# Kronuz/Xapiand

Hardware: AMD Instinct MI355X
Metric: queries/sec + p50 latency, 10M-doc synthetic index, 3-term AND, top-10 (higher is better)
Workload: dtype u32 postings + f64 BM25

## Files before the change

### include/xgm.h

```cpp
#ifndef XGM_H
#define XGM_H

#include <stddef.h>
#include <stdint.h>

#ifdef __cplusplus
extern "C" {
#endif
#if defined(__GNUC__)
#pragma GCC visibility push(default)
#endif

#define XGM_MAX_TERMS 16
#define XGM_MAX_K 1024

#define XGM_OK 0
#define XGM_UNSUPPORTED 1
#define XGM_E_INVALID (-1)
#define XGM_E_IO (-2)
#define XGM_E_NO_DEVICE (-3)
#define XGM_E_DEVICE (-4)
#define XGM_E_REVISION (-5)
#define XGM_E_NOMEM (-6)

// ... 326 lines not shown
void xgm_batch_release(xgm_inflight*);

int xgm_merge_shards_device(xgm_index*, const void* d_all_hits, const void* d_all_hdrs,
                            uint32_t n_shards, uint32_t nq, uint32_t k_stride, const uint32_t* k,
                            void* d_out_hits, void* d_out_hdrs);

size_t xgm_shard_record_bytes(uint32_t nq, uint32_t k_stride);
int xgm_merge_shards_packed_device(xgm_index*, const void* d_all_records, uint32_t n_shards, uint32_t nq, uint32_t k_stride,
                                   const uint32_t* k, void* d_out_hits, void* d_out_hdrs);

int xgm_search_sharded(xgm_index* const* shards, uint32_t n_shards, const xgm_query_desc* descs,
                       uint32_t nq, uint32_t k_stride, xgm_hit* hits, xgm_result_hdr* hdrs);

int xgm_debug_sharded_info(const xgm_index* shards0, uint64_t* out4);

int xgm_index_set_near_colocated(xgm_index*, int may_exist);

int xgm_index_set_profiling(xgm_index*, int on);
double xgm_last_kernel_ms(const xgm_index*);
const char* xgm_last_kernel_name(const xgm_index*);

#define XGM_TRAFFIC_FIELDS 10
int xgm_last_batch_traffic(xgm_index*, uint64_t* out, uint32_t n);

uint64_t xgm_query_postings_bytes(const xgm_index*, const xgm_query*);

int64_t xgm_debug_decode_term_device(xgm_index*, uint32_t term_id, uint32_t* did, uint32_t* wdf, uint64_t cap);

int64_t xgm_debug_read_doclen(xgm_index*, uint32_t* out, uint64_t cap);

int64_t xgm_debug_read_positions(xgm_index*, uint32_t term_id, uint32_t* out, uint64_t cap);

int64_t xgm_debug_read_container(xgm_index*, uint32_t term_id, uint32_t stripe, unsigned char* out, uint64_t cap, uint32_t* layout);

int xgm_debug_read_wdf_summary(xgm_index*, uint32_t term_id, uint32_t stripe, uint64_t* out);

int xgm_debug_read_term_wdf0(xgm_index*, uint32_t term_id, uint32_t* out);

int64_t xgm_debug_read_flat(xgm_index*, uint32_t term_id, uint32_t* did, unsigned char* wdf, uint32_t* pos, uint64_t cap, uint32_t* has_pos);

double xgm_debug_plan_us(const xgm_index*, const xgm_query_desc* descs, const xgm_global_stats* gs, uint32_t nq, uint32_t reps);

int xgm_debug_batch_launches(const xgm_index*, const xgm_query* qs, uint32_t nq, char* out, uint32_t cap);

int xgm_debug_host_ns(uint64_t* out8);

// ... 32 lines not shown
```

### xapiand_amd/_lib.py

```python
import ctypes as C
import os

XGM_MAX_TERMS = 16
XGM_MAX_TREE = 40
XGM_OP_TREE = 8
XGM_MAX_K = 1024
XGM_OK, XGM_UNSUPPORTED = 0, 1
XGM_E_INVALID, XGM_E_IO, XGM_E_NO_DEVICE, XGM_E_DEVICE, XGM_E_REVISION, XGM_E_NOMEM = -1, -2, -3, -4, -5, -6
XGM_OP_AND, XGM_OP_OR, XGM_OP_PHRASE = 1, 2, 3
XGM_OP_AND_NOT, XGM_OP_AND_MAYBE, XGM_OP_FILTER, XGM_OP_NEAR = 4, 5, 6, 7
XGM_REPLAY_BATCH_COUNT = 2
XGM_REPLAY_BATCH_FROZEN = 1
XGM_KNOWN_LOWER_BOUND = 1 << 63
XGM_ALL_NOT_A_MATCH = 0x80000000
XGM_MATCHES_LOWER_BOUND = 1 << 63
XGM_DEVICE_NONE = -1
UINT64_MAX = (1 << 64) - 1

_HERE = os.path.dirname(os.path.abspath(__file__))
LIB_PATH = os.environ.get("XGM_LIB_PATH") or os.path.join(_HERE, "csrc", "libxgm.so")


class RawPostings(C.Structure):
    _fields_ = [("n_terms", C.c_uint32), ("lastdocid", C.c_uint32), ("doccount", C.c_uint32),
# ... 156 lines not shown
    ("xgm_debug_replay_list", C.c_int, [C.c_int, _P(Hit), C.c_uint64, C.c_uint32, C.c_uint64, C.c_uint32, C.c_uint64, _P(Hit), _P(ReplayFigures)]),
    ("xgm_debug_batch_replay_info", C.c_int, [_P(C.c_uint64)]),
    ("xgm_search_batch", C.c_int, [C.c_void_p, _P(Query), C.c_uint32, C.c_uint32, _P(Hit), _P(ResultHdr)]),
    ("xgm_search_batch_known", C.c_int, [C.c_void_p, _P(Query), C.c_uint32, C.c_uint32, _P(Hit), _P(ResultHdr), _P(C.c_uint64)]),
    ("xgm_search_batch_begin", C.c_int, [C.c_void_p, _P(Query), C.c_uint32, C.c_uint32, _P(C.c_void_p)]),
    ("xgm_get_mset_batch_begin", C.c_int, [C.c_void_p, _P(QueryDesc), _P(GlobalStats), C.c_uint32, C.c_uint32, _P(C.c_void_p)]),
    ("xgm_batch_end", C.c_int, [C.c_void_p, _P(_P(Hit)), _P(_P(ResultHdr))]),
    ("xgm_batch_known", C.c_int, [C.c_void_p, _P(_P(C.c_uint64))]),
    ("xgm_batch_poll", C.c_int, [C.c_void_p]),
    ("xgm_batch_release", None, [C.c_void_p]),
    ("xgm_search_batch_device", C.c_int, [C.c_void_p, _P(Query), C.c_uint32, C.c_uint32, C.c_void_p, C.c_void_p]),
    ("xgm_get_mset_batch", C.c_int, [C.c_void_p, _P(QueryDesc), _P(GlobalStats), C.c_uint32, C.c_uint32, _P(Hit), _P(ResultHdr)]),
    ("xgm_get_mset_batch_device", C.c_int, [C.c_void_p, _P(QueryDesc), _P(GlobalStats), C.c_uint32, C.c_uint32, C.c_void_p, C.c_void_p]),
    ("xgm_search_sharded", C.c_int, [_P(C.c_void_p), C.c_uint32, _P(QueryDesc), C.c_uint32, C.c_uint32, _P(Hit), _P(ResultHdr)]),
    ("xgm_debug_sharded_info", C.c_int, [C.c_void_p, _P(C.c_uint64)]),
    ("xgm_merge_shards_device", C.c_int, [C.c_void_p, C.c_void_p, C.c_void_p, C.c_uint32, C.c_uint32, C.c_uint32, _P(C.c_uint32), C.c_void_p, C.c_void_p]),
    ("xgm_merge_shards_packed_device", C.c_int, [C.c_void_p, C.c_void_p, C.c_uint32, C.c_uint32, C.c_uint32, _P(C.c_uint32), C.c_void_p, C.c_void_p]),
    ("xgm_shard_record_bytes", C.c_size_t, [C.c_uint32, C.c_uint32]),
    ("xgm_index_set_profiling", C.c_int, [C.c_void_p, C.c_int]),
    ("xgm_index_set_near_colocated", C.c_int, [C.c_void_p, C.c_int]),
    ("xgm_last_kernel_ms", C.c_double, [C.c_void_p]),
    ("xgm_last_kernel_name", C.c_char_p, [C.c_void_p]),
    ("xgm_last_batch_traffic", C.c_int, [C.c_void_p, _P(C.c_uint64), C.c_uint32]),
    ("xgm_query_postings_bytes", C.c_uint64, [C.c_void_p, _P(Query)]),
    ("xgm_debug_decode_term_device", C.c_int64, [C.c_void_p, C.c_uint32, _P(C.c_uint32), _P(C.c_uint32), C.c_uint64]),
    ("xgm_debug_read_doclen", C.c_int64, [C.c_void_p, _P(C.c_uint32), C.c_uint64]),
    ("xgm_debug_read_positions", C.c_int64, [C.c_void_p, C.c_uint32, _P(C.c_uint32), C.c_uint64]),
    ("xgm_debug_read_container", C.c_int64, [C.c_void_p, C.c_uint32, C.c_uint32, _P(C.c_ubyte), C.c_uint64, _P(C.c_uint32)]),
    ("xgm_debug_read_wdf_summary", C.c_int, [C.c_void_p, C.c_uint32, C.c_uint32, _P(C.c_uint64)]),
    ("xgm_debug_read_term_wdf0", C.c_int, [C.c_void_p, C.c_uint32, _P(C.c_uint32)]),
    ("xgm_debug_read_flat", C.c_int64, [C.c_void_p, C.c_uint32, _P(C.c_uint32), _P(C.c_ubyte), _P(C.c_uint32), C.c_uint64, _P(C.c_uint32)]),
    ("xgm_debug_plan_us", C.c_double, [C.c_void_p, _P(QueryDesc), _P(GlobalStats), C.c_uint32, C.c_uint32]),
    ("xgm_debug_batch_launches", C.c_int, [C.c_void_p, _P(Query), C.c_uint32, C.c_char_p, C.c_uint32]),
    ("xgm_index_set_batching", C.c_int, [C.c_void_p, C.c_uint32]),
    ("xgm_debug_batching_info", C.c_int, [C.c_void_p, _P(C.c_uint64)]),
    ("xgm_debug_host_ns", C.c_int, [_P(C.c_uint64)]),
    ("xgm_debug_concurrent_searches", C.c_double, [C.c_void_p, _P(QueryDesc), _P(GlobalStats), C.c_uint32, C.c_uint32, C.c_uint32, C.c_uint32, _P(C.c_double)]),
    ("xgm_debug_phase_cycles", C.c_int, [_P(C.c_ulonglong)]),
    ("xgm_debug_merge_cycles", C.c_int, [_P(C.c_ulonglong)]),
    ("xgm_debug_orw_phase_cycles", C.c_int, [_P(C.c_ulonglong)]),
    ("xgm_debug_plan_batch", C.c_int64, [C.c_void_p, _P(Query), C.c_uint32, C.c_char_p, _P(C.c_uint32), C.c_uint64]),
    ("xgm_debug_or_bounds", C.c_int, [C.c_void_p, _P(Query), _P(C.c_double), _P(C.c_double), _P(C.c_double)]),
    ("xgm_debug_last_units", C.c_int64, [C.c_void_p, _P(C.c_ulonglong), C.c_uint64]),
    ("xgm_debug_last_units2", C.c_int64, [C.c_void_p, _P(C.c_ulonglong), _P(C.c_ulonglong), C.c_uint64]),
    ("xgm_mset_bounds_known", None, [_P(Query), _P(ResultHdr), C.c_uint64, _P(C.c_uint32), _P(C.c_uint32), _P(C.c_uint32)]),
    ("xgm_index_attach_column_ordinals", C.c_int, [C.c_void_p, C.c_uint32, _P(C.c_uint32), C.c_uint32, C.c_uint32]),
# ... 51 lines not shown
```

### xapiand_amd/csrc/xgm_api.cc

```cpp
#include <hip/hip_runtime.h>

#include <algorithm>
#include <atomic>
#include <chrono>
#include <condition_variable>
#include <deque>
#include <thread>
#include <cstdarg>
#include <cstdlib>
#include <cmath>
#include <cstring>
#include <string>

#include "xgm_filter_hold.h"
#include "xgm_internal.h"
#include "xgm_launch.h"

int xgm_read_segment_file(const char* path, XgmSegmentBlob* blob);


static thread_local char g_err[512] = "";

int xgm_set_error(int code, const char* fmt, ...) {
    va_list ap;
// ... 168 lines not shown
    return XGM_OK;
}


void xgm_shard_ctx_destroy(XgmShardCtx* c);
void xgm_batcher_destroy(xgm_index* idx);

static void fill_view(xgm_index* idx) {
    xgm_seg_dev& v = idx->view;
    v.doclen = (const uint32_t*)idx->d_sections[XGM_S_DOCLEN];
    v.term_blk = (const uint64_t*)idx->d_sections[XGM_S_TERM_BLK];
    v.term_word = (const uint64_t*)idx->d_sections[XGM_S_TERM_WORD];
    v.term_pos = (const uint64_t*)idx->d_sections[XGM_S_TERM_POS];
    v.blk_first = (const uint32_t*)idx->d_sections[XGM_S_BLK_FIRST];
    v.blk_meta = (const uint32_t*)idx->d_sections[XGM_S_BLK_META];
    v.blk_word = (const uint32_t*)idx->d_sections[XGM_S_BLK_WORD];
    v.blk_pos = (const uint32_t*)idx->d_sections[XGM_S_BLK_POS];
    v.words = (const uint32_t*)idx->d_sections[XGM_S_WORDS];
    v.positions = (const unsigned char*)idx->d_sections[XGM_S_POSITIONS];
    v.term_flags = (const uint32_t*)idx->d_sections[XGM_S_TERM_FLAGS];
    v.stripe_bits = idx->hdr.stripe_bits;
    v.lastdocid = idx->hdr.lastdocid;
    v.dense_id = nullptr; v.dense_dir = nullptr; v.dense_data = nullptr; v.n_dense = 0; v.dense_pos = 0; v.dense_plane = 0;
    v.dense_p2 = nullptr; v.bit_screen = 0; v.exact_wdf = 0; v.dense_wdf0 = nullptr; v.reserved_ = 0;
    v.doclen_narrow = nullptr; v.doclen_narrow_bits = 0; v.doclen_base = 0;
    v.flat_off = nullptr; v.flat_did = nullptr; v.flat_wdf = nullptr; v.flat_pos = nullptr;
    v.n_stripes = (idx->hdr.lastdocid >> idx->hdr.stripe_bits) + 1u;
}

static void adopt_host_dictionary(xgm_index* idx, const XgmSegmentBlob& blob) {
    const xgm_seg_header* h = blob.header();
    const uint32_t T = h->n_terms;
    idx->term_df.assign(blob.section<uint32_t>(XGM_S_TERM_DF), blob.section<uint32_t>(XGM_S_TERM_DF) + T);
    idx->term_cf.assign(blob.section<uint32_t>(XGM_S_TERM_CF), blob.section<uint32_t>(XGM_S_TERM_CF) + T);
    idx->term_wdfub.assign(blob.section<uint32_t>(XGM_S_TERM_WDFUB), blob.section<uint32_t>(XGM_S_TERM_WDFUB) + T);
    idx->term_flags.assign(blob.section<uint32_t>(XGM_S_TERM_FLAGS), blob.section<uint32_t>(XGM_S_TERM_FLAGS) + T);
    idx->term_blk.assign(blob.section<uint64_t>(XGM_S_TERM_BLK), blob.section<uint64_t>(XGM_S_TERM_BLK) + T + 1);
    idx->term_word.assign(blob.section<uint64_t>(XGM_S_TERM_WORD), blob.section<uint64_t>(XGM_S_TERM_WORD) + T + 1);
    idx->str_off.assign(blob.section<uint64_t>(XGM_S_STR_OFF), blob.section<uint64_t>(XGM_S_STR_OFF) + T + 1);
    const char* sb = blob.section<char>(XGM_S_STR_BYTES);
    idx->str_bytes.assign(sb, sb + h->sec_bytes[XGM_S_STR_BYTES]);
}

extern "C" int xgm_index_open(const char* segment_path, int device, uint64_t revision, xgm_index** out) {
    if (!segment_path || !out) return xgm_set_error(XGM_E_INVALID, "null argument");
    *out = nullptr;
    XgmSegmentBlob blob;
// ... 769 lines not shown
    const uint64_t t_up = now_ns();
    g_host_ns[5] += t_up - t_cp;
    unsigned char* din = (unsigned char*)s->d_in;
    s->d_queries = (xgm_dev_query*)(din + o_dq);
    s->d_maxposs = (double*)(din + o_mp);
    s->d_work = (xgm_work*)(din + o_wk);
    s->d_kq = (uint32_t*)(din + o_kq);
    s->d_goff = (uint32_t*)(din + o_go);

    xgm_match_launch L;
    L.seg = idx->view;
    L.queries = s->d_queries;
    L.nq = nq; L.n_work = bp.n_work; L.work = s->d_work; L.stripes_per_group = bp.stripes_per_group; L.sub_bits = bp.sub_bits;
    static const bool debug_units = getenv("XGM_DEBUG_UNITS") != nullptr;
    if (debug_units && nq > 1) { g_last_work = bp.work; g_last_ghdr = s->d_ghdr; }
    L.tab_terms = bp.tab_terms; L.cap = bp.cap; L.k_stride = bp.k_stride_c;
    L.phrase = bp.phrase; L.wide = bp.wide; L.sided = bp.andw ? bp.sided : 0; L.orw2 = bp.orw2; L.orw_planes = bp.orw_planes; L.or_flat = bp.or_flat;
    L.tally = idx->tally;
    L.cand = s->d_cand; L.ghdr = s->d_ghdr;
    hipEvent_t pe0 = nullptr, pe1 = nullptr;
    if ((rc = next_event_pair(idx, &pe0, &pe1))) return rc;
    idx->last_kernel = all ? "xgm_andw_all_kernel" : list ? "xgm_andw_list_kernel" : dense ? "xgm_dense_kernel" : bp.andw ? "xgm_andw_kernel" : bp.orw2 ? "xgm_orw2_kernel" : bp.orw ? "xgm_orw_kernel" : bp.and_only ? "xgm_and_kernel" : "xgm_match_kernel";
    idx->last_ghdr = s->d_ghdr; idx->last_n_work = bp.n_work;
    if (bp.orw || (bp.andw && bp.phrase)) {
        if (!hist_zeroed) {
            const size_t n_hist = list ? (size_t)bp.n_work : (size_t)nq * XGM_OR_HIST;
            if ((rc = grow(&s->d_hist, &s->cap_hist, n_hist))) return rc;
            HIP_TRY(hipMemsetAsync(s->d_hist, 0, n_hist * 4, stream));
        }
        L.hist = s->d_hist;
    }
    if (fused || list) L.fuse = (const xgm_fuse*)(din + o_fu);
    static const bool ext_launch = getenv("XGM_NO_EXT_LAUNCH") == nullptr;
    const bool ext = ext_launch && !dense && (bp.andw || (bp.orw && !bp.orw2));
    s->last_stop = nullptr;
    if (ext) {
        L.ev_start = pe0;
        L.ev_stop = pe1 ? pe1 : (fused ? s->ev1 : nullptr);
        if (fused) s->last_stop = L.ev_stop;
        pe0 = pe1 = nullptr;
    }
    if (pe0) HIP_TRY(hipEventRecord(pe0, stream));
    if ((rc = all ? xgm_launch_andw_all(L, all_out, stream) : list ? xgm_launch_andw_list(L, stream) : dense ? xgm_launch_dense(L, stream) : bp.andw ? xgm_launch_andw(L, stream)
              : bp.orw ? xgm_launch_orw(L, s->d_hist, stream)
              : bp.and_only ? xgm_launch_and(L, stream) : xgm_launch_match(L, stream)))
        return rc;
// ... 2255 lines not shown
    }
    return (int64_t)n;
}

extern "C" int xgm_last_batch_traffic(xgm_index* idx, uint64_t* out, uint32_t n) {
    if (!idx || !out) return xgm_set_error(XGM_E_INVALID, "null argument");
    uint64_t t[XGM_TRAFFIC_FIELDS] = {};
    if (!idx->last_ghdr || idx->last_n_work == 0) return xgm_set_error(XGM_E_INVALID, "no batch has run on this index");
    int rc = use_device(idx->device);
    if (rc) return rc;
    HIP_TRY(hipDeviceSynchronize());
    std::vector<xgm_group_hdr> h(idx->last_n_work);
    HIP_TRY(hipMemcpy(h.data(), idx->last_ghdr, h.size() * sizeof(xgm_group_hdr), hipMemcpyDeviceToHost));
    const bool list = idx->last_kernel && !strcmp(idx->last_kernel, "xgm_andw_list_kernel");
    for (const xgm_group_hdr& g : h) {
        t[0] += g.c_bmp_words; t[1] += g.c_probes; t[2] += g.c_blk_words; t[3] += g.c_hdrs;
        t[4] += g.c_doclen; t[5] += g.c_aux_words; t[6] += list ? (g.n_cand * 3u + 1u) / 2u : g.n_cand; t[7] += list ? g.c_pad[1] : g.c_pos;
        t[8] += g.c_probes_raw; t[9] += g.c_doclen_raw;
    }
    for (uint32_t i = 0; i < n && i < XGM_TRAFFIC_FIELDS; ++i) out[i] = t[i];
    return XGM_OK;
}

extern "C" double xgm_debug_plan_us(const xgm_index* idx, const xgm_query_desc* descs, const xgm_global_stats* gs, uint32_t nq, uint32_t reps) {
    if (!idx || !descs || nq == 0 || reps == 0) return -1.0;
    xgm_query q;
    const auto t0 = std::chrono::steady_clock::now();
    for (uint32_t r = 0; r < reps; ++r)
        for (uint32_t i = 0; i < nq; ++i)
            if (xgm_plan_query(idx, &descs[i], gs ? &gs[i] : nullptr, &q) < 0) return -1.0;
    const double us = std::chrono::duration<double, std::micro>(std::chrono::steady_clock::now() - t0).count();
    return us / ((double)nq * reps);
}

int xgm_phase_cycles_fetch(unsigned long long* out8);
extern "C" int xgm_debug_phase_cycles(unsigned long long* out8) { return xgm_phase_cycles_fetch(out8); }
int xgm_orw_cycles_fetch(unsigned long long* out8);
int xgm_merge_cycles_fetch(unsigned long long* out8);
extern "C" int xgm_debug_merge_cycles(unsigned long long* out8) { return xgm_merge_cycles_fetch(out8); }
extern "C" int xgm_debug_orw_phase_cycles(unsigned long long* out8) { return xgm_orw_cycles_fetch(out8); }

extern "C" int64_t xgm_debug_plan_batch(const xgm_index* idx, const xgm_query* qs, uint32_t nq, char* kernel, uint32_t* units, uint64_t cap) {
    if (!idx || !qs || !kernel || (!units && cap)) return xgm_set_error(XGM_E_INVALID, "null argument");
    if (nq == 0) return 0;
    std::vector<xgm_dev_query> dq(nq);
    std::vector<uint32_t> kq(nq);
// ... 61 lines not shown
```

### xapiand_amd/csrc/xgm_dense.hip

```cpp
#include <hip/hip_runtime.h>

#include <algorithm>
#include <cstdlib>
#include <vector>

#include "xgm_device.h"
#include "xgm_internal.h"
#include "xgm_launch.h"

namespace {

#define DN_TRY(expr)                                                                            \
    do {                                                                                        \
        hipError_t e_ = (expr);                                                                 \
        if (e_ != hipSuccess) { rc = xgm_launch_error(#expr, (int)e_, hipGetErrorString(e_)); goto fail; } \
    } while (0)

constexpr uint32_t kStage = 272;

__device__ __forceinline__ uint32_t dn_extract(const uint32_t* s, uint32_t idx, uint32_t bw) {
    uint32_t bit = idx * bw, w = bit >> 5;
    uint32_t v = __builtin_amdgcn_alignbit(s[w + 1], s[w], bit & 31u);
    return bw >= 32u ? v : (v & ((1u << bw) - 1u));
}
// ... 204 lines not shown
    idx->view.flat_wdf = (const unsigned char*)idx->d_flat_wdf;
    idx->view.flat_pos = (const uint32_t*)idx->d_flat_pos;
    idx->flat_postings = n;
    idx->flat_bytes = off.size() * 8 + n * (idx->d_flat_pos ? 9 : 5) + 768;
    idx->device_bytes += idx->flat_bytes;
    return XGM_OK;
fail:
    if (d_terms) hipFree(d_terms);
    for (void** p : {&idx->d_flat_off, &idx->d_flat_did, &idx->d_flat_wdf, &idx->d_flat_pos}) if (*p) { hipFree(*p); *p = nullptr; }
    return rc;
}

static int build_containers(xgm_index* idx);

int xgm_build_dense(xgm_index* idx) {
    if (int rc_ = build_narrow_doclen(idx)) return rc_;
    if (int rc_ = build_containers(idx)) return rc_;
    return build_flat(idx);
}

static int build_containers(xgm_index* idx) {
    idx->view.dense_id = nullptr; idx->view.dense_dir = nullptr; idx->view.dense_data = nullptr;
    idx->view.n_dense = 0; idx->view.dense_plane = 0; idx->view.dense_p2 = nullptr; idx->view.bit_screen = 0;
    idx->view.exact_wdf = 0; idx->view.dense_wdf0 = nullptr; idx->view.reserved_ = 0;
    if (idx->d_dense_p2) { hipFree(idx->d_dense_p2); idx->d_dense_p2 = nullptr; }
    if (idx->d_dense_wdf0) { hipFree(idx->d_dense_wdf0); idx->d_dense_wdf0 = nullptr; }
    idx->term_wdfmax.clear();
    const uint32_t SB = idx->hdr.stripe_bits;
    const uint32_t n_stripes = (idx->hdr.lastdocid >> SB) + 1u;
    idx->view.n_stripes = n_stripes;
    if (getenv("XGM_NO_DENSE")) return XGM_OK;
    const uint32_t NW = (1u << SB) / 32u;
    const int with_pos = idx->hdr.has_positions ? 1 : 0;
    const uint32_t min_avg = getenv("XGM_DENSE_MIN_AVG") ? (uint32_t)atoi(getenv("XGM_DENSE_MIN_AVG")) : XGM_DENSE_MIN_AVG;
    std::vector<uint32_t> dense_terms;
    std::vector<uint32_t> dense_id(idx->hdr.n_terms, 0xFFFFFFFFu);
    uint32_t max_blocks = 1;
    for (uint32_t t = 0; t < idx->hdr.n_terms; ++t) {
        if ((uint64_t)idx->term_df[t] >= (uint64_t)min_avg * n_stripes && idx->term_wdfub[t] <= 254u) {
            dense_id[t] = (uint32_t)dense_terms.size();
            dense_terms.push_back(t);
            max_blocks = std::max<uint32_t>(max_blocks, (uint32_t)(idx->term_blk[t + 1] - idx->term_blk[t]));
        }
    }
    const uint32_t n_dense = (uint32_t)dense_terms.size();
    if (n_dense == 0) return XGM_OK;
    int rc = XGM_OK;
// ... 36 lines not shown
        if (idx->d_dense_wdf0) { hipFree(idx->d_dense_wdf0); idx->d_dense_wdf0 = nullptr; }
    }
    hipLaunchKernelGGL(k_dense_fill, dim3(n_stripes, n_dense), dim3(256), 0, 0, idx->view, d_terms, n_stripes, (const uint32_t*)idx->d_dense_dir,
                       (unsigned char*)idx->d_dense_data, with_pos, d_wmax, (unsigned long long*)idx->d_dense_p2, (uint32_t*)idx->d_dense_wdf0);
    DN_TRY(hipGetLastError());
    DN_TRY(hipDeviceSynchronize());
    wmax.resize(n_dense);
    DN_TRY(hipMemcpy(wmax.data(), d_wmax, (size_t)n_dense * 4, hipMemcpyDeviceToHost));
    idx->term_wdfmax.assign(idx->term_wdfub.begin(), idx->term_wdfub.end());
    for (uint32_t d = 0; d < n_dense; ++d)
        if (wmax[d] && wmax[d] < idx->term_wdfmax[dense_terms[d]]) idx->term_wdfmax[dense_terms[d]] = wmax[d];
    idx->dense_bytes = dense_id.size() * 4 + dir.size() * 4 + units * 16 + (idx->d_dense_p2 ? dir.size() * 8 : 0) + (idx->d_dense_wdf0 ? (size_t)n_dense * 4 : 0);
    idx->device_bytes += idx->dense_bytes;
    idx->view.dense_id = (const uint32_t*)idx->d_dense_id;
    idx->view.dense_dir = (const uint32_t*)idx->d_dense_dir;
    idx->view.dense_data = (const unsigned char*)idx->d_dense_data;
    idx->view.n_dense = n_dense;
    idx->view.dense_pos = (uint32_t)with_pos;
    idx->view.dense_plane = plane_off;
    idx->view.dense_p2 = (const unsigned long long*)idx->d_dense_p2;
    idx->view.bit_screen = getenv("XGM_NO_BIT_SCREEN") ? 0u : 1u;
    idx->view.dense_wdf0 = (const uint32_t*)idx->d_dense_wdf0;
    idx->view.exact_wdf = (!getenv("XGM_NO_EXACT_WDF") && idx->d_dense_wdf0 && idx->d_dense_p2 && plane_off && 5u + SB <= 28u) ? 1u : 0u;
    idx->dense_min_df = (uint64_t)min_avg * n_stripes;
    hipFree(d_terms); hipFree(d_cnt); hipFree(d_wmax);
    return XGM_OK;
fail:
    if (d_terms) hipFree(d_terms);
    if (d_cnt) hipFree(d_cnt);
    if (d_wmax) hipFree(d_wmax);
    if (idx->d_dense_id) { hipFree(idx->d_dense_id); idx->d_dense_id = nullptr; }
    if (idx->d_dense_dir) { hipFree(idx->d_dense_dir); idx->d_dense_dir = nullptr; }
    if (idx->d_dense_data) { hipFree(idx->d_dense_data); idx->d_dense_data = nullptr; }
    if (idx->d_dense_p2) { hipFree(idx->d_dense_p2); idx->d_dense_p2 = nullptr; }
    if (idx->d_dense_wdf0) { hipFree(idx->d_dense_wdf0); idx->d_dense_wdf0 = nullptr; }
    idx->view.dense_p2 = nullptr; idx->view.dense_wdf0 = nullptr; idx->view.exact_wdf = 0;
    return rc;
}
```

### xapiand_amd/csrc/xgm_dense_body.inc

```

constexpr uint32_t kDenseT = 4;
constexpr uint32_t kDenseSpg = 32;
constexpr uint32_t kDenseCap = 128;
constexpr uint32_t kDenseRing = 256;
#ifndef XGM_DENSE_PREFILTER_MIN
#define XGM_DENSE_PREFILTER_MIN 48
#endif
constexpr uint32_t kDensePrefilterMin = XGM_DENSE_PREFILTER_MIN;
#ifndef XGM_DENSE_EXACT_MIN
#define XGM_DENSE_EXACT_MIN XGM_DENSE_PREFILTER_MIN
#endif
constexpr uint32_t kDenseExactMin = XGM_DENSE_EXACT_MIN;
constexpr uint32_t kDenseExactLane = 16;

#ifndef XGM_DENSE_WORD_MAJOR
#define XGM_DENSE_WORD_MAJOR 1
#endif
#ifndef XGM_DENSE_GATHER_ALL
#define XGM_DENSE_GATHER_ALL 2
#endif
constexpr uint32_t kDenseGatherAll = XGM_DENSE_GATHER_ALL;
#ifndef XGM_DENSE_REFILL
#define XGM_DENSE_REFILL 64
#endif
constexpr uint32_t kDenseRefill = XGM_DENSE_REFILL;
#ifndef XGM_DENSE_PIPE
#define XGM_DENSE_PIPE 1
#endif
constexpr uint32_t kDensePipe = XGM_DENSE_PIPE;
#ifndef XGM_DENSE_HIST_EVERY
#define XGM_DENSE_HIST_EVERY 2
#endif
constexpr uint32_t kDenseHistEvery = XGM_DENSE_HIST_EVERY;
constexpr uint32_t kDenseSq = 128;

constexpr size_t kDenseCoreBytes = (size_t)kDenseCap * 8 + (size_t)kDenseCap * 4 + (size_t)kDenseT * kDenseSpg * 4 + (size_t)kDenseRing * 4;
constexpr size_t kDenseP2Bytes = (size_t)kDenseSpg * kDenseT * 8;
constexpr size_t kDenseXcBytes = 64 * 8;
static_assert(4u * kDenseExactLane == 64u, "a lane's packed code is one u64");
__host__ __device__ constexpr size_t dense_wave_bytes(bool phrase, uint32_t terms = kDenseT) {
    return kDenseCoreBytes + (phrase ? (size_t)kDenseSq * 16 + (size_t)terms * kPosFast * 64 * 2 : kDenseP2Bytes + kDenseXcBytes);
}

typedef uint32_t dense_u4 __attribute__((ext_vector_type(4)));

struct PrefixList {
    xgm_prefix_entry* out;
    uint32_t cap, n;
    bool done, has_first, hold;
    uint64_t first_w, hold_w;
    uint32_t hold_did, hold_idx;
    uint32_t* cnt_all; uint32_t u_first, u_mine, calls;
    bool count_all;
    __device__ __forceinline__ void init(xgm_prefix_entry* o, uint32_t c, uint32_t* counters, uint32_t first_slot, uint32_t my_slot, bool all) {
        out = o; cap = c; n = 0; done = false; has_first = false; hold = false; first_w = hold_w = 0; hold_did = hold_idx = 0;
        cnt_all = all ? nullptr : counters; u_first = first_slot; u_mine = my_slot; calls = 0; count_all = all;
    }
    __device__ __forceinline__ void put(uint32_t idx, uint64_t w, uint64_t nw, uint32_t did, uint32_t has_next) {
        xgm_prefix_entry e; e.wbits = w; e.next_wbits = nw; e.did = did; e.has_next = has_next;
        out[idx] = e;
    }
    __device__ __forceinline__ void look_back(uint32_t lane) {
        if (!cnt_all || done) return;
        uint32_t sum = 0;
        for (uint32_t v0 = u_first; v0 < u_mine && sum < cap; v0 += 64u) {
            const uint32_t v = v0 + lane;
            uint32_t c = 0;
// ... 125 lines not shown
    }

    uint64_t* tk_w = reinterpret_cast<uint64_t*>(base);
    uint32_t* tk_d = reinterpret_cast<uint32_t*>(base + (size_t)kDenseCap * 8);
    uint32_t* rs = reinterpret_cast<uint32_t*>(base + (size_t)kDenseCap * 12);
    uint32_t* ring = reinterpret_cast<uint32_t*>(base + (size_t)kDenseCap * 12 + (size_t)kDenseT * kDenseSpg * 4);
    uint64_t* sq_w = reinterpret_cast<uint64_t*>(base + kDenseCoreBytes);
    uint32_t* sq_d = reinterpret_cast<uint32_t*>(base + kDenseCoreBytes + (size_t)kDenseSq * 8);
    uint32_t* sq_v = sq_d + kDenseSq;
    uint16_t* lpos = reinterpret_cast<uint16_t*>(sq_v + kDenseSq);
    uint32_t* p2s = reinterpret_cast<uint32_t*>(base + kDenseCoreBytes);
    unsigned long long* xcs = reinterpret_cast<unsigned long long*>(base + kDenseCoreBytes + kDenseP2Bytes);
    bool use_p2 = false;
    if constexpr (!PHRASE) use_p2 = seg.dense_p2 != nullptr;
    bool use_exact = false;
    if constexpr (!PHRASE) use_exact = use_p2 && rfl32(seg.exact_wdf) != 0u;
    uint32_t z_mask = 0xFu;

    const uint32_t s_begin = wk.s_begin, s_end = wk.s_end;
    const bool empty = (q.flags & XGM_QF_EMPTY) || s_begin >= s_end || k == 0;
    const uint32_t n_local = empty ? 0u : (s_end - s_begin < kDenseSpg ? s_end - s_begin : kDenseSpg);

    uint32_t cn_bmpw = 0, cn_probe = 0, cn_dl = 0, cn_aux = 0, cn_probe_raw = 0, cn_dl_raw = 0, q_cands = 0;
    unsigned long long cn_pos = 0;
    auto tally_sectors = [&](bool valid, uint32_t key, uint32_t sh) {
        const uint32_t prev = (uint32_t)__shfl_up((int)key, 1);
        return (uint32_t)__popcll(__ballot(valid && (lane == 0u || (prev >> sh) != (key >> sh))));
    };

#pragma unroll
    for (uint32_t i = 0; i < kDenseCap; i += 64u) { tk_w[i + lane] = 0; tk_d[i + lane] = 0xFFFFFFFFu; }
#pragma unroll
    for (uint32_t i = 0; i < kDenseT * kDenseSpg; i += 64u) {
        const uint32_t e = i + lane, t = e / kDenseSpg, x = e % kDenseSpg;
        uint32_t off = 0;
        unsigned long long p2w = 0;
        if (t < T && x < n_local) {
            const uint32_t id = q.term_id[t];
            const uint32_t dn = id != 0xFFFFFFFFu ? seg.dense_id[id] : 0xFFFFFFFFu;
            if (dn != 0xFFFFFFFFu) off = seg.dense_dir[(size_t)dn * seg.n_stripes + (s_begin + x)];
            if constexpr (!PHRASE) { if (use_p2 && dn != 0xFFFFFFFFu) p2w = seg.dense_p2[(size_t)dn * seg.n_stripes + (s_begin + x)]; }
        }
        rs[x * kDenseT + t] = off;
        if constexpr (!PHRASE) { if (use_p2) { p2s[x * (2u * kDenseT) + t] = (uint32_t)p2w; p2s[x * (2u * kDenseT) + kDenseT + t] = (uint32_t)(p2w >> 32); } }
    }
    if (TALLY) { cn_aux += T * n_local * (use_p2 ? 3u : 1u); }
// ... 86 lines not shown
            v.w = lane + 192u < NW ? w[lane + 192u] : 0u;
        } else {
            v = reinterpret_cast<const dense_u4*>(p)[lane * 4u < NW ? lane : 0u];
            if (lane * 4u >= NW) v = dense_u4{0u, 0u, 0u, 0u};
        }
        return v;
    };
    auto load_and = [&](uint32_t x) {
        dense_u4 r[kDenseT];
#pragma unroll
        for (uint32_t t = 0; t < kDenseT; ++t) {
            const uint32_t off = off_of(t, x);
            r[t] = load_words(seg.dense_data + (size_t)off * 16);
        }
        dense_u4 a = r[0] & r[1] & r[2] & r[3];
        if (LIST && part_mask) {
            if (!(part_mask & 1u)) a.x = 0u;
            if (!(part_mask & 2u)) a.y = 0u;
            if (!(part_mask & 4u)) a.z = 0u;
            if (!(part_mask & 8u)) a.w = 0u;
        }
        if (TALLY) { cn_bmpw += T * NW; }
        return a;
    };

    auto make_room = [&]() {
        if (__builtin_expect(tkn + 64u > kDenseCap || (PHRASE && !theta_valid && tkn >= k), 0)) {
            dense_topk_sort(tk_w, tk_d, PHRASE ? lane : dense_sort_lane(lane));
            tkn = tkn < k ? tkn : k;
            if (tkn == k) { theta_valid = true; theta_w = tk_w[k - 1]; theta_d = tk_d[k - 1]; }
#pragma unroll
            for (uint32_t i = 0; i < kDenseCap; i += 64u) if (i + lane >= tkn) { tk_w[i + lane] = 0; tk_d[i + lane] = 0xFFFFFFFFu; }
            wave_lds_fence();
        }
    };
    auto insert = [&](bool take, uint64_t wb, uint32_t did) {
        const uint64_t tm = __ballot(take);
        if (take) { const uint32_t p = tkn + mbcnt(tm); tk_w[p] = wb; tk_d[p] = did; }
        tkn += (uint32_t)__popcll(tm);
        wave_lds_fence();
    };

    uint32_t sq_n = 0;
    uint32_t n_tested = 0;
    auto survivors = [&](uint32_t n) {
        const uint32_t k0 = XGM_CLK();
// ... 259 lines not shown
            } else {
                const uint32_t sec = tally_sectors(valid, did, 6u);
                cn_probe += T * sec; cn_probe_raw += T * n;
            }
            cn_dl += tally_sectors(valid, did, dl_bits == 8u ? 6u : dl_bits == 16u ? 5u : 4u); cn_dl_raw += n;
        }
        const uint32_t c_b = XGM_CLK();
        weigh();
        const uint32_t c_c = XGM_CLK();
        if (PHRASE) {
            if (hc_requested) { hc_requested = false; hc_pending = true; }
            else if (hist_g && (n_rounds++ & (kDenseHistEvery - 1u)) == 0u) request_histogram();
        }
        q_n[kDensePipe - 1u] = n; q_did[kDensePipe - 1u] = did; q_dlen[kDensePipe - 1u] = dlen;
#pragma unroll
        for (uint32_t t = 0; t < kDenseT; ++t) q_wv[kDensePipe - 1u][t] = wv[t];
        const uint32_t c_d = XGM_CLK();
        ck_i += (c_b - c_a) + (c_d - c_c); ck_w += c_c - c_b;
    };

    uint32_t sl = next_q(0);
    dense_u4 m = dense_u4{0u, 0u, 0u, 0u}, m_next = dense_u4{0u, 0u, 0u, 0u};
    uint32_t sl_next = n_local;
    if (sl < n_local) {
        m = load_and(sl);
        sl_next = next_q(sl + 1u);
        if (sl_next < n_local) m_next = load_and(sl_next);
    }
    uint32_t o = 0u, o1 = 0u, o2 = 0u, o3 = 0u, n_total = 0u, done = 0u, tail = 0u;
    bool fresh = true;
    while ((sl < n_local || pend) && !(LIST && pf.done)) {
        const uint32_t c_p0 = XGM_CLK();
        if (sl < n_local && pend < kDenseRefill) {
            unsigned long long xcode = ~0ull; (void)xcode;
            if constexpr (!PHRASE) { if (use_exact && !fresh) xcode = xcs[lane]; }
            if (fresh) {
                uint32_t cnt = (uint32_t)(__popc(m.x) + __popc(m.y) + __popc(m.z) + __popc(m.w));
                uint64_t th_bits = theta_valid ? theta_w : 0ull;
                if (PHRASE && theta_glob > th_bits) th_bits = theta_glob;
                {
                    if (!PHRASE) matches += cnt;
                    dense_u4 b2[kDenseT];
                    bool have_b2 = false, exact_stripe = false, have_total = false;
                    uint32_t total = 0u;
                    if constexpr (!PHRASE) {
                        if (use_exact) {
                            total = rl32(wave_incl_scan(cnt), 63); have_total = true;
                            exact_stripe = total >= kDenseExactMin;
                            if (exact_stripe) {
#pragma unroll
// ... 83 lines not shown
                    ring[(wbase + O) & (kDenseRing - 1u)] = dbase + (D) + bit;                            \
                }                                                                                         \
                MW &= MW - 1u;                                                                            \
                ++O;                                                                                      \
            }
            if (kWordMajor) {
                XGM_DENSE_EMIT(m.x, o, 0u)
                XGM_DENSE_EMIT(m.y, o1, 2048u)
                XGM_DENSE_EMIT(m.z, o2, 4096u)
                XGM_DENSE_EMIT(m.w, o3, 6144u)
            } else {
                XGM_DENSE_EMIT(m.x, o, 0u)
                XGM_DENSE_EMIT(m.y, o, 32u)
                XGM_DENSE_EMIT(m.z, o, 64u)
                XGM_DENSE_EMIT(m.w, o, 96u)
            }
#undef XGM_DENSE_EMIT
            if constexpr (!PHRASE) { if (use_exact && done + take_n != n_total) xcs[lane] = xcode; }
            tail = (tail + take_n) & (kDenseRing - 1u);
            pend += take_n;
            if (TALLY) { q_cands += take_n; }
            done = lim;
            if (done == n_total) {
                sl = sl_next;
                m = m_next;
                if (sl < n_local) {
                    sl_next = next_q(sl + 1u);
                    if (sl_next < n_local) m_next = load_and(sl_next);
                }
                fresh = true;
            }
            wave_lds_fence();
        }
        ck_p += XGM_CLK() - c_p0;
        if (pend >= 64u || (sl >= n_local && pend)) issue(pend < 64u ? pend : 64u);
    }
#pragma unroll
    for (uint32_t i = 0; i < kDensePipe; ++i) if (!(LIST && pf.done)) weigh();
    if (PHRASE) { while (sq_n && !(LIST && pf.done)) { const uint32_t s0 = XGM_CLK(); survivors(sq_n < 64u ? sq_n : 64u); ck_s += XGM_CLK() - s0; } }
    if (LIST) {
        pf.finish(lane);
        for (int sh = 32; sh > 0; sh >>= 1) matches += (uint32_t)__shfl_xor((int)matches, sh);
        unsigned long long cn_pos_sum = cn_pos;
        if (TALLY) { for (int sh = 32; sh > 0; sh >>= 1) cn_pos_sum += (unsigned long long)__shfl_xor((long long)cn_pos_sum, sh); }
        if (lane == 0) {
            xgm_group_hdr h = {};
            h.matches = (unsigned long long)matches | (pf.done ? XGM_MATCHES_LOWER_BOUND : 0ull);
            h.n_cand = pf.n < pf.cap ? pf.n : pf.cap;
            h.pad = (pf.has_first ? XGM_PFX_HAS_FIRST : 0u) | (pf.done ? 0u : XGM_PFX_COMPLETE);
            h.t_start = t_unit_start; h.t_end = __builtin_readcyclecounter();
            h.c_pos = pf.first_w;
// ... 8 lines not shown
        }
        return;
    }

    dense_topk_sort(tk_w, tk_d, PHRASE ? lane : dense_sort_lane(lane));
    for (int sh = 32; sh > 0; sh >>= 1) matches += (uint32_t)__shfl_xor((int)matches, sh);
    if (PHRASE) { for (int sh = 32; sh > 0; sh >>= 1) n_tested += (uint32_t)__shfl_xor((int)n_tested, sh); }
    if (PHRASE && TALLY) { for (int sh = 32; sh > 0; sh >>= 1) cn_pos += (unsigned long long)__shfl_xor((long long)cn_pos, sh); }
    const bool any_pruned = PHRASE && __ballot(pos_pruned) != 0ull;
    const uint32_t n_out = tkn < k ? tkn : k;
    xgm_cand* out = cand_out + (size_t)wk.slot * k_stride;
    const bool through = fuse != nullptr;
    for (uint32_t i = lane; i < n_out; i += 64u) {
        xgm_cand c;
        c.wbits = tk_w[i]; c.did = tk_d[i]; c.subqs = (uint32_t)__popc(q.score_mask);
        xgm_store_cand(through, &out[i], c);
    }
    if (lane == 0) {
        xgm_group_hdr h;
        h.matches = (unsigned long long)matches | (any_pruned ? XGM_MATCHES_LOWER_BOUND : 0ull); h.n_cand = n_out; h.pad = TALLY ? q_cands : (PHRASE ? n_tested : 0u);
        h.t_start = t_unit_start; h.t_end = __builtin_readcyclecounter();
        h.c_pos = cn_pos; h.c_bmp_words = cn_bmpw; h.c_probes = cn_probe; h.c_blk_words = 0; h.c_hdrs = 0;
        h.c_doclen = cn_dl; h.c_aux_words = cn_aux; h.c_probes_raw = cn_probe_raw; h.c_doclen_raw = cn_dl_raw; h.c_pad[0] = 0; h.c_pad[1] = 0;
        if (ALL) { h.matches = al.n; h.c_pad[0] = al.c; h.c_pad[1] = al.overflow ? XGM_ALL_OVERFLOW : 0u; }
#ifdef XGM_DENSE_CLOCKS
        h.c_pad[0] = ck_p; h.c_pad[1] = ck_i; h.c_pos = (unsigned long long)(ck_w - ck_s_in) | ((unsigned long long)ck_s << 32);
#if XGM_DENSE_CLOCKS == 2
        h.c_pad[0] = sk_a; h.c_pad[1] = sk_b; h.c_pos = (unsigned long long)sk_c | ((unsigned long long)sk_d << 32); h.pad = n_tested | (sk_calls << 20);
#endif
#endif
        xgm_store_hdr(through, &ghdr_out[wk.slot], h);
    }
    if (through) xgm_unit_arrive<false>(*fuse, wk.qi, k, (uint32_t)__popc(q.score_mask), tk_w, tk_d, nullptr, kDenseCap, cand_out, ghdr_out, k_stride, lane,
                           [&]() { dense_topk_sort(tk_w, tk_d, PHRASE ? lane : dense_sort_lane(lane)); });
}
```

### xapiand_amd/csrc/xgm_internal.h

```cpp
#ifndef XGM_INTERNAL_H
#define XGM_INTERNAL_H

#include <atomic>
#include <cstdarg>
#include <cstdint>
#include <cstdio>
#include <map>
#include <mutex>
#include <string>
#include <utility>
#include <vector>

#include "../../include/xgm.h"
#include "xgm_segment.h"

int xgm_set_error(int code, const char* fmt, ...) __attribute__((format(printf, 2, 3)));

struct XgmSegmentBlob {
    std::vector<uint8_t> bytes;
    const uint8_t* map = nullptr;
    size_t map_size = 0;
    XgmSegmentBlob() = default;
    XgmSegmentBlob(const XgmSegmentBlob&) = delete;
    XgmSegmentBlob& operator=(const XgmSegmentBlob&) = delete;
// ... 57 lines not shown
    xgm_seg_dev view{};
    uint64_t device_bytes = 0;
    void* d_dense_id = nullptr;
    void* d_dense_dir = nullptr;
    void* d_dense_data = nullptr;
    void* d_dense_p2 = nullptr;
    void* d_dense_wdf0 = nullptr;
    void* d_doclen_narrow = nullptr;
    void* d_flat_off = nullptr;
    void* d_flat_did = nullptr;
    void* d_flat_wdf = nullptr;
    void* d_flat_pos = nullptr;
    uint64_t flat_bytes = 0, flat_postings = 0;
    uint64_t dense_bytes = 0;
    uint64_t dense_min_df = UINT64_MAX;
    void* stream = nullptr;
    bool own_stream = false;
    bool profiling = false;
    std::atomic<bool> near_colocated{false};
    bool tally = false;
    const char* last_kernel = "";
    void* last_ghdr = nullptr;
    uint32_t last_n_work = 0;
    std::vector<std::pair<void*, void*>> prof_events;
    size_t prof_used = 0;
    std::mutex scratch_mu;
    std::vector<XgmScratch*> scratch_pool;
    uint32_t scratch_total = 0;
    XgmBatcher* batcher = nullptr;
    XgmShardCtx* shard_ctx = nullptr;
    std::vector<XgmShardCtx*> retired_shard_ctx;
    std::map<uint32_t, std::pair<void*, uint32_t>> columns;
    std::vector<uint32_t> term_order;
    std::once_flag term_order_once;
    std::vector<void*> retired_columns;
    std::mutex columns_mu;
    struct ListColumn { void* head = nullptr; void* ext = nullptr; uint32_t n_distinct = 0; };
    std::map<uint32_t, ListColumn> list_columns;
    std::mutex live_mu;
    void* d_live = nullptr;
    uint32_t live_state = 0;
    uint32_t live_source = 0;
    uint32_t live_launches = 0;
    uint64_t live_marked = 0;
};

// ... 6 lines not shown
```

### xapiand_amd/csrc/xgm_segment.h

```cpp
#ifndef XGM_SEGMENT_H
#define XGM_SEGMENT_H

#include <stdint.h>

#define XGM_SEG_MAGIC "XGMSEG1"
#define XGM_SEG_VERSION 2u
#define XGM_BLOCK 128u
#define XGM_DEFAULT_STRIPE_BITS 13u
#define XGM_MIN_STRIPE_BITS 8u
#define XGM_MAX_STRIPE_BITS 13u
#define XGM_WORD_PAD 8u

#define XGM_META(count, bwg, bww) (((count)-1u) | ((uint32_t)(bwg) << 8) | ((uint32_t)(bww) << 16))
#define XGM_META_COUNT(m) (((m)&0xFFu) + 1u)
#define XGM_META_BWG(m) (((m) >> 8) & 0xFFu)
#define XGM_META_BWW(m) (((m) >> 16) & 0xFFu)

#define XGM_TF_POS_OK 1u
#define XGM_TF_POS16 2u
#define XGM_POS_PAD 32u

enum xgm_section {
    XGM_S_DOCLEN = 0,
    XGM_S_TERM_DF,
// ... 36 lines not shown
    const uint32_t* blk_pos;
    const uint32_t* words;
    const unsigned char* positions;
    const uint32_t* term_flags;
    uint32_t stripe_bits;
    uint32_t lastdocid;
    const uint32_t* dense_id;
    const uint32_t* dense_dir;
    const unsigned char* dense_data;
    uint32_t n_dense;
    uint32_t n_stripes;
    uint32_t dense_pos;
    const unsigned char* doclen_narrow;
    uint32_t doclen_narrow_bits, doclen_base;
    uint32_t dense_plane;
    const uint64_t* flat_off;
    const uint32_t* flat_did;
    const unsigned char* flat_wdf;
    const uint32_t* flat_pos;
    const unsigned long long* dense_p2;
    uint32_t bit_screen;
    uint32_t exact_wdf;
    const uint32_t* dense_wdf0;
    unsigned long long reserved_;
} xgm_seg_dev;

#define XGM_DENSE_MIN_AVG 32u

static inline uint32_t xgm_bits_needed(uint32_t v) {
    uint32_t b = 0;
    while (v) { ++b; v >>= 1; }
    return b;
}

#endif
```

Measured before the change: 952,500.

## Stage dense bitmap AND loads to skip later terms when first two are empty

Splits the dense-kernel bitmap AND into two stages. The first two term bitmaps are loaded and ANDed, and the third and fourth are fetched only when that partial AND is nonzero for the lane. The staged loads are pipelined one stripe ahead, replacing the previous single load_and prefetch. The aim is to cut memory reads for selective conjunctions, at the cost of an extra dependency between loads, more registers, and lower memory-level parallelism. A tally counter and an API to read the skipped words are added for diagnostics.

```diff
diff --git a/include/xgm.h b/include/xgm.h
--- a/include/xgm.h
+++ b/include/xgm.h
@@ -372,6 +372,7 @@
 
 #define XGM_TRAFFIC_FIELDS 10
 int xgm_last_batch_traffic(xgm_index*, uint64_t* out, uint32_t n);
+int xgm_last_batch_bitmap_skipped(xgm_index*, uint64_t* words);
 
 uint64_t xgm_query_postings_bytes(const xgm_index*, const xgm_query*);
 
diff --git a/xapiand_amd/_lib.py b/xapiand_amd/_lib.py
--- a/xapiand_amd/_lib.py
+++ b/xapiand_amd/_lib.py
@@ -202,6 +202,7 @@
     ("xgm_last_kernel_ms", C.c_double, [C.c_void_p]),
     ("xgm_last_kernel_name", C.c_char_p, [C.c_void_p]),
     ("xgm_last_batch_traffic", C.c_int, [C.c_void_p, _P(C.c_uint64), C.c_uint32]),
+    ("xgm_last_batch_bitmap_skipped", C.c_int, [C.c_void_p, _P(C.c_uint64)]),
     ("xgm_query_postings_bytes", C.c_uint64, [C.c_void_p, _P(Query)]),
     ("xgm_debug_decode_term_device", C.c_int64, [C.c_void_p, C.c_uint32, _P(C.c_uint32), _P(C.c_uint32), C.c_uint64]),
     ("xgm_debug_read_doclen", C.c_int64, [C.c_void_p, _P(C.c_uint32), C.c_uint64]),
diff --git a/xapiand_amd/csrc/xgm_api.cc b/xapiand_amd/csrc/xgm_api.cc
--- a/xapiand_amd/csrc/xgm_api.cc
+++ b/xapiand_amd/csrc/xgm_api.cc
@@ -214,7 +214,7 @@
     v.stripe_bits = idx->hdr.stripe_bits;
     v.lastdocid = idx->hdr.lastdocid;
     v.dense_id = nullptr; v.dense_dir = nullptr; v.dense_data = nullptr; v.n_dense = 0; v.dense_pos = 0; v.dense_plane = 0;
-    v.dense_p2 = nullptr; v.bit_screen = 0; v.exact_wdf = 0; v.dense_wdf0 = nullptr; v.reserved_ = 0;
+    v.dense_p2 = nullptr; v.bit_screen = 0; v.exact_wdf = 0; v.dense_wdf0 = nullptr; v.staged_bitmaps = 0; v.reserved_ = 0;
     v.doclen_narrow = nullptr; v.doclen_narrow_bits = 0; v.doclen_base = 0;
     v.flat_off = nullptr; v.flat_did = nullptr; v.flat_wdf = nullptr; v.flat_pos = nullptr;
     v.n_stripes = (idx->hdr.lastdocid >> idx->hdr.stripe_bits) + 1u;
@@ -1030,6 +1030,13 @@
     if ((rc = next_event_pair(idx, &pe0, &pe1))) return rc;
     idx->last_kernel = all ? "xgm_andw_all_kernel" : list ? "xgm_andw_list_kernel" : dense ? "xgm_dense_kernel" : bp.andw ? "xgm_andw_kernel" : bp.orw2 ? "xgm_orw2_kernel" : bp.orw ? "xgm_orw_kernel" : bp.and_only ? "xgm_and_kernel" : "xgm_match_kernel";
     idx->last_ghdr = s->d_ghdr; idx->last_n_work = bp.n_work;
+    idx->last_tallied = idx->tally;
+    if (idx->tally) {
+        idx->last_staged_slots.clear();
+        if (mode == 0 && bp.andw && !bp.phrase)
+            for (uint32_t i = 0; i < bp.n_work; ++i)
+                if (h_dq[bp.work[i].qi].flags & XGM_QF_DENSE) idx->last_staged_slots.push_back(bp.work[i].slot);
+    }
     if (bp.orw || (bp.andw && bp.phrase)) {
         if (!hist_zeroed) {
             const size_t n_hist = list ? (size_t)bp.n_work : (size_t)nq * XGM_OR_HIST;
@@ -3331,6 +3338,22 @@
     return XGM_OK;
 }
 
+extern "C" int xgm_last_batch_bitmap_skipped(xgm_index* idx, uint64_t* words) {
+    if (!idx || !words) return xgm_set_error(XGM_E_INVALID, "null argument");
+    if (!idx->last_ghdr || idx->last_n_work == 0) return xgm_set_error(XGM_E_INVALID, "no batch has run on this index");
+    if (!idx->last_tallied) return xgm_set_error(XGM_E_INVALID, "the last batch did not run the tallying instantiation");
+    int rc = use_device(idx->device);
+    if (rc) return rc;
+    HIP_TRY(hipDeviceSynchronize());
+    std::vector<xgm_group_hdr> h(idx->last_n_work);
+    HIP_TRY(hipMemcpy(h.data(), idx->last_ghdr, h.size() * sizeof(xgm_group_hdr), hipMemcpyDeviceToHost));
+    uint64_t sum = 0;
+    for (uint32_t slot : idx->last_staged_slots)
+        if (slot < h.size()) sum += h[slot].c_pad[0];
+    *words = sum;
+    return XGM_OK;
+}
+
 extern "C" double xgm_debug_plan_us(const xgm_index* idx, const xgm_query_desc* descs, const xgm_global_stats* gs, uint32_t nq, uint32_t reps) {
     if (!idx || !descs || nq == 0 || reps == 0) return -1.0;
     xgm_query q;
diff --git a/xapiand_amd/csrc/xgm_dense.hip b/xapiand_amd/csrc/xgm_dense.hip
--- a/xapiand_amd/csrc/xgm_dense.hip
+++ b/xapiand_amd/csrc/xgm_dense.hip
@@ -250,7 +250,7 @@
 static int build_containers(xgm_index* idx) {
     idx->view.dense_id = nullptr; idx->view.dense_dir = nullptr; idx->view.dense_data = nullptr;
     idx->view.n_dense = 0; idx->view.dense_plane = 0; idx->view.dense_p2 = nullptr; idx->view.bit_screen = 0;
-    idx->view.exact_wdf = 0; idx->view.dense_wdf0 = nullptr; idx->view.reserved_ = 0;
+    idx->view.exact_wdf = 0; idx->view.dense_wdf0 = nullptr; idx->view.staged_bitmaps = 0; idx->view.reserved_ = 0;
     if (idx->d_dense_p2) { hipFree(idx->d_dense_p2); idx->d_dense_p2 = nullptr; }
     if (idx->d_dense_wdf0) { hipFree(idx->d_dense_wdf0); idx->d_dense_wdf0 = nullptr; }
     idx->term_wdfmax.clear();
@@ -333,6 +333,7 @@
     idx->view.bit_screen = getenv("XGM_NO_BIT_SCREEN") ? 0u : 1u;
     idx->view.dense_wdf0 = (const uint32_t*)idx->d_dense_wdf0;
     idx->view.exact_wdf = (!getenv("XGM_NO_EXACT_WDF") && idx->d_dense_wdf0 && idx->d_dense_p2 && plane_off && 5u + SB <= 28u) ? 1u : 0u;
+    idx->view.staged_bitmaps = getenv("XGM_NO_STAGED_BITMAPS") ? 0u : 1u;
     idx->dense_min_df = (uint64_t)min_avg * n_stripes;
     hipFree(d_terms); hipFree(d_cnt); hipFree(d_wmax);
     return XGM_OK;
diff --git a/xapiand_amd/csrc/xgm_dense_body.inc b/xapiand_amd/csrc/xgm_dense_body.inc
--- a/xapiand_amd/csrc/xgm_dense_body.inc
+++ b/xapiand_amd/csrc/xgm_dense_body.inc
@@ -43,6 +43,7 @@
 }
 
 typedef uint32_t dense_u4 __attribute__((ext_vector_type(4)));
+struct dense_u4x2 { dense_u4 a, b; };
 
 struct PrefixList {
     xgm_prefix_entry* out;
@@ -214,6 +215,7 @@
     const uint32_t n_local = empty ? 0u : (s_end - s_begin < kDenseSpg ? s_end - s_begin : kDenseSpg);
 
     uint32_t cn_bmpw = 0, cn_probe = 0, cn_dl = 0, cn_aux = 0, cn_probe_raw = 0, cn_dl_raw = 0, q_cands = 0;
+    uint32_t cn_skip = 0;
     unsigned long long cn_pos = 0;
     auto tally_sectors = [&](bool valid, uint32_t key, uint32_t sh) {
         const uint32_t prev = (uint32_t)__shfl_up((int)key, 1);
@@ -346,6 +348,30 @@
         }
         if (TALLY) { cn_bmpw += T * NW; }
         return a;
+    };
+    const dense_u4 kOnes = dense_u4{0xFFFFFFFFu, 0xFFFFFFFFu, 0xFFFFFFFFu, 0xFFFFFFFFu};
+    bool staged = false;
+    if constexpr (!PHRASE) staged = rfl32(seg.staged_bitmaps) != 0u;
+    auto stage1 = [&](uint32_t x) {
+        dense_u4x2 r;
+        r.a = dense_u4{0u, 0u, 0u, 0u}; r.b = kOnes;
+        const bool in = lane * 4u < NW;
+        const uint32_t o0 = off_of(0u, x), o1 = off_of(1u, x);
+        if (in) r.a = reinterpret_cast<const dense_u4*>(seg.dense_data + (size_t)o0 * 16)[lane];
+        if (T >= 2u && in) r.b = reinterpret_cast<const dense_u4*>(seg.dense_data + (size_t)o1 * 16)[lane];
+        if (TALLY) { cn_bmpw += T * NW; }
+        return r;
+    };
+    auto stage2 = [&](uint32_t x, const dense_u4 a01) {
+        dense_u4x2 r;
+        r.a = kOnes; r.b = kOnes;
+        const bool in = lane * 4u < NW;
+        const bool want = in && (!staged || (a01.x | a01.y | a01.z | a01.w) != 0u);
+        const uint32_t o2 = off_of(2u, x), o3 = off_of(3u, x);
+        if (T >= 3u && want) r.a = reinterpret_cast<const dense_u4*>(seg.dense_data + (size_t)o2 * 16)[lane];
+        if (T >= 4u && want) r.b = reinterpret_cast<const dense_u4*>(seg.dense_data + (size_t)o3 * 16)[lane];
+        if (TALLY) { if (T >= 3u) cn_skip += 4u * (T - 2u) * (uint32_t)__popcll(__ballot(in && !want)); }
+        return r;
     };
 
     auto make_room = [&]() {
@@ -651,10 +677,32 @@
     uint32_t sl = next_q(0);
     dense_u4 m = dense_u4{0u, 0u, 0u, 0u}, m_next = dense_u4{0u, 0u, 0u, 0u};
     uint32_t sl_next = n_local;
-    if (sl < n_local) {
-        m = load_and(sl);
-        sl_next = next_q(sl + 1u);
-        if (sl_next < n_local) m_next = load_and(sl_next);
+    dense_u4 n2 = kOnes, n3 = kOnes, f0 = dense_u4{0u, 0u, 0u, 0u}, f1 = dense_u4{0u, 0u, 0u, 0u};
+    uint32_t sl_s1 = n_local;
+    (void)n2; (void)n3; (void)f0; (void)f1; (void)sl_s1; (void)load_and; (void)stage1; (void)stage2;
+    auto shift_in = [&]() {
+        m_next = f0 & f1;
+        const dense_u4x2 r = stage2(sl_next, m_next);
+        n2 = r.a; n3 = r.b;
+        sl_s1 = next_q(sl_next + 1u);
+        if (sl_s1 < n_local) { const dense_u4x2 f = stage1(sl_s1); f0 = f.a; f1 = f.b; }
+    };
+    if constexpr (PHRASE) {
+        if (sl < n_local) {
+            m = load_and(sl);
+            sl_next = next_q(sl + 1u);
+            if (sl_next < n_local) m_next = load_and(sl_next);
+        }
+    } else {
+        if (sl < n_local) {
+            const dense_u4x2 e = stage1(sl);
+            sl_next = next_q(sl + 1u);
+            if (sl_next < n_local) { const dense_u4x2 f = stage1(sl_next); f0 = f.a; f1 = f.b; }
+            m = e.a & e.b;
+            const dense_u4x2 l = stage2(sl, m);
+            if (sl_next < n_local) shift_in();
+            m &= l.a & l.b;
+        }
     }
     uint32_t o = 0u, o1 = 0u, o2 = 0u, o3 = 0u, n_total = 0u, done = 0u, tail = 0u;
     bool fresh = true;
@@ -784,11 +832,18 @@
             if (TALLY) { q_cands += take_n; }
             done = lim;
             if (done == n_total) {
-                sl = sl_next;
-                m = m_next;
-                if (sl < n_local) {
-                    sl_next = next_q(sl + 1u);
-                    if (sl_next < n_local) m_next = load_and(sl_next);
+                if constexpr (PHRASE) {
+                    sl = sl_next;
+                    m = m_next;
+                    if (sl < n_local) {
+                        sl_next = next_q(sl + 1u);
+                        if (sl_next < n_local) m_next = load_and(sl_next);
+                    }
+                } else {
+                    sl = sl_next;
+                    m = m_next & n2 & n3;
+                    sl_next = sl_s1;
+                    if (sl_next < n_local) shift_in();
                 }
                 fresh = true;
             }
@@ -843,6 +898,7 @@
         h.t_start = t_unit_start; h.t_end = __builtin_readcyclecounter();
         h.c_pos = cn_pos; h.c_bmp_words = cn_bmpw; h.c_probes = cn_probe; h.c_blk_words = 0; h.c_hdrs = 0;
         h.c_doclen = cn_dl; h.c_aux_words = cn_aux; h.c_probes_raw = cn_probe_raw; h.c_doclen_raw = cn_dl_raw; h.c_pad[0] = 0; h.c_pad[1] = 0;
+        if (!PHRASE && TALLY) h.c_pad[0] = cn_skip;
         if (ALL) { h.matches = al.n; h.c_pad[0] = al.c; h.c_pad[1] = al.overflow ? XGM_ALL_OVERFLOW : 0u; }
 #ifdef XGM_DENSE_CLOCKS
         h.c_pad[0] = ck_p; h.c_pad[1] = ck_i; h.c_pos = (unsigned long long)(ck_w - ck_s_in) | ((unsigned long long)ck_s << 32);
diff --git a/xapiand_amd/csrc/xgm_internal.h b/xapiand_amd/csrc/xgm_internal.h
--- a/xapiand_amd/csrc/xgm_internal.h
+++ b/xapiand_amd/csrc/xgm_internal.h
@@ -103,6 +103,8 @@
     const char* last_kernel = "";
     void* last_ghdr = nullptr;
     uint32_t last_n_work = 0;
+    bool last_tallied = false;
+    std::vector<uint32_t> last_staged_slots;
     std::vector<std::pair<void*, void*>> prof_events;
     size_t prof_used = 0;
     std::mutex scratch_mu;
diff --git a/xapiand_amd/csrc/xgm_segment.h b/xapiand_amd/csrc/xgm_segment.h
--- a/xapiand_amd/csrc/xgm_segment.h
+++ b/xapiand_amd/csrc/xgm_segment.h
@@ -82,7 +82,8 @@
     uint32_t bit_screen;
     uint32_t exact_wdf;
     const uint32_t* dense_wdf0;
-    unsigned long long reserved_;
+    uint32_t staged_bitmaps;
+    uint32_t reserved_;
 } xgm_seg_dev;
 
 #define XGM_DENSE_MIN_AVG 32u
```

Result: faster. 973,600 (median of 6 runs) (+2.2%).
